# cipherflow-fhe/lattisense

Measured on AMD Instinct MI355X. Metric: ckks_hmult_relin_rescale_throughput, higher is better.
Workload: dtype u64

## Files before the change

### include/lattisense_amd.h

```cpp
#ifndef LATTISENSE_AMD_H
#define LATTISENSE_AMD_H
#include <stddef.h>
#include <stdint.h>

#ifdef __cplusplus
extern "C" {
#endif

typedef struct lsa_context_st* lsa_context;
typedef struct lsa_key_st* lsa_key;

enum { LSA_OK = 0, LSA_ERR_ARG = 1, LSA_ERR_NO_DEVICE = 2, LSA_ERR_HIP = 3, LSA_ERR_INTERNAL = 4 };
enum { LSA_ALGO_BFV = 0, LSA_ALGO_CKKS = 1 };

const char* lsa_last_error(void);
const char* lsa_version(void);
const char* lsa_build_flags(void);

int lsa_context_create(int algo, int n, const uint64_t* q, int nq, const uint64_t* p, int np, uint64_t t,
                       int device, lsa_context* out);
int lsa_context_destroy(lsa_context ctx);
int lsa_context_moduli(lsa_context ctx, uint64_t* out, int capacity, int* count);

int lsa_malloc(lsa_context ctx, void** dptr, size_t bytes);
// ... 79 lines not shown
                       void* stream);
int lsa_bfv_mult_sum(lsa_context ctx, int level, int n, const uint64_t* const* as, const long long* sas, const uint64_t* const* bs,
                     const long long* sbs, const uint64_t* addend, long long s_addend, uint64_t* d3, int batch, long long sd,
                     void* stream);
int lsa_bfv_dot(lsa_context ctx, int level, int n, const uint64_t* const* as, const long long* sas, const uint64_t* const* bs,
                const long long* sbs, const uint64_t* addend, long long s_addend, lsa_key rlk, uint64_t* out, int batch,
                long long sout, void* stream);
int lsa_bfv_dot_plan(int n_ring, const uint64_t* q, int nq, int level, int terms, int* max_terms, int* n_groups, int* aux_limbs);

int lsa_set_bfv_dot_chunk(lsa_context ctx, int pairs);
int lsa_set_tile_batch(lsa_context ctx, int tile_batch);
int lsa_set_fp64_ntt(lsa_context ctx, int enable);
int lsa_set_dual_stream(lsa_context ctx, int enable);
int lsa_set_fuse_tails(lsa_context ctx, int enable);
int lsa_set_modup_lift(lsa_context ctx, int enable);
int lsa_set_ks_tail_in_mac(lsa_context ctx, int mode);
int lsa_set_rescale_head_in_conv(lsa_context ctx, int mode);
int lsa_set_ntt_chunk_mib(lsa_context ctx, int mib);
int lsa_ckks_rotate_many(lsa_context ctx, int level, const uint64_t* in, int n_rot, const uint64_t* galois_elements,
                         const lsa_key* glk, uint64_t* const* outs, int batch, long long sin, long long sout, void* stream);
int lsa_bfv_rotate_many(lsa_context ctx, int level, const uint64_t* in, int n_rot, const uint64_t* galois_elements,
                        const lsa_key* glk, uint64_t* const* outs, int batch, long long sin, long long sout, void* stream);

typedef struct lsa_bootstrap_st* lsa_bootstrap;
int lsa_bootstrap_create(lsa_context ctx, int cts_depth, int stc_depth, int k, int double_angle, double message_ratio,
                         double in_scale, double out_scale, int log_slots, void* stream, lsa_bootstrap* out);
int lsa_bootstrap_create_ex(lsa_context ctx, int cts_depth, int stc_depth, int k, int double_angle, double message_ratio,
                            double in_scale, double out_scale, int log_slots, int sine_deg, int arcsine_deg, void* stream,
                            lsa_bootstrap* out);
int lsa_bootstrap_evalmod_constants(lsa_bootstrap b, int* n_cheb, double* cheb, int* n_asin, double* asin_coef);
// ... 115 lines not shown
```

### lattisense_amd/_native.py

```python
import ctypes
import importlib.util
import os

_HERE = os.path.dirname(os.path.abspath(__file__))
LIB_PATH = os.environ.get("LSA_NATIVE_LIB") or os.path.join(_HERE, "liblattisense_amd.so")

_lib = None

c_u64p = ctypes.POINTER(ctypes.c_uint64)
c_ll = ctypes.c_longlong
c_vp = ctypes.c_void_p
c_int = ctypes.c_int


class LsaError(RuntimeError):
    def __init__(self, code, msg):
        super().__init__("lattisense_amd error %d: %s" % (code, msg))
        self.code = code


def _preload_hip_runtime():
    spec = importlib.util.find_spec("torch")
    if spec is not None and spec.origin:
        p = os.path.join(os.path.dirname(spec.origin), "lib", "libamdhip64.so")
# ... 54 lines not shown
    "lsa_bfv_rotate": (c_int, [c_vp, c_int, c_vp, ctypes.c_uint64, c_vp, c_vp, c_int, c_ll, c_ll, c_vp]),
    "lsa_bfv_rescale": (c_int, [c_vp, c_int, c_int, c_vp, c_vp, c_int, c_ll, c_ll, c_vp]),
    "lsa_bfv_mult_relin": (c_int, [c_vp, c_int, c_vp, c_vp, c_vp, c_vp, c_int, c_ll, c_ll, c_ll, c_vp]),
    "lsa_bfv_mult_sum": (c_int, [c_vp, c_int, c_int, ctypes.POINTER(c_vp), ctypes.POINTER(c_ll), ctypes.POINTER(c_vp),
                                 ctypes.POINTER(c_ll), c_vp, c_ll, c_vp, c_int, c_ll, c_vp]),
    "lsa_bfv_dot": (c_int, [c_vp, c_int, c_int, ctypes.POINTER(c_vp), ctypes.POINTER(c_ll), ctypes.POINTER(c_vp), ctypes.POINTER(c_ll),
                            c_vp, c_ll, c_vp, c_vp, c_int, c_ll, c_vp]),
    "lsa_bfv_dot_plan": (c_int, [c_int, c_u64p, c_int, c_int, c_int, ctypes.POINTER(c_int), ctypes.POINTER(c_int),
                                 ctypes.POINTER(c_int)]),
    "lsa_set_bfv_dot_chunk": (c_int, [c_vp, c_int]),
    "lsa_set_tile_batch": (c_int, [c_vp, c_int]),
    "lsa_set_fp64_ntt": (c_int, [c_vp, c_int]),
    "lsa_set_dual_stream": (c_int, [c_vp, c_int]),
    "lsa_set_fuse_tails": (c_int, [c_vp, c_int]),
    "lsa_set_modup_lift": (c_int, [c_vp, c_int]),
    "lsa_set_ks_tail_in_mac": (c_int, [c_vp, c_int]),
    "lsa_set_rescale_head_in_conv": (c_int, [c_vp, c_int]),
    "lsa_set_ntt_chunk_mib": (c_int, [c_vp, c_int]),
    "lsa_debug_set_ntt_stamps": (c_int, [c_vp, c_vp]),
    "lsa_debug_baseconv_plans": (c_int, [c_vp, c_int, ctypes.POINTER(c_int), ctypes.POINTER(c_int), ctypes.POINTER(c_int),
                                         ctypes.POINTER(c_int)]),
    "lsa_debug_key_switch_fused": (c_int, [c_vp, c_int, c_vp, ctypes.POINTER(c_int)]),
    "lsa_ckks_rotate_many": (c_int, [c_vp, c_int, c_vp, c_int, c_u64p, ctypes.POINTER(c_vp), ctypes.POINTER(c_vp), c_int,
                                     ctypes.c_longlong, ctypes.c_longlong, c_vp]),
    "lsa_bfv_rotate_many": (c_int, [c_vp, c_int, c_vp, c_int, c_u64p, ctypes.POINTER(c_vp), ctypes.POINTER(c_vp), c_int,
                                    ctypes.c_longlong, ctypes.c_longlong, c_vp]),
    "lsa_bfv_mult_plain_mul": (c_int, [c_vp, c_int, c_vp, c_vp, c_vp, c_int, c_ll, c_ll, c_ll, c_vp]),
    "lsa_bfv_mac_plain_mul": (c_int, [c_vp, c_int, c_int, ctypes.POINTER(c_vp), ctypes.POINTER(c_ll), ctypes.POINTER(c_vp),
                                      ctypes.POINTER(c_ll), c_vp, c_ll, c_vp, c_int, c_ll, c_vp]),
    "lsa_bfv_rotate_mac_plain_mul": (c_int, [c_vp, c_int, c_vp, c_int, c_u64p, ctypes.POINTER(c_vp), ctypes.POINTER(c_vp),
# ... 112 lines not shown
```

### lattisense_amd/build.py

```python
import importlib.util
import os
import subprocess
import sys

HERE = os.path.dirname(os.path.abspath(__file__))
CSRC = os.path.join(HERE, "csrc")
LIB = os.path.join(HERE, "liblattisense_amd.so")
HIP_SOURCES = ["kernels.hip", "context.hip", "key_switch.hip", "ops.hip", "linear_transform.hip", "bfv_encode.hip", "bfv_plain.hip", "slot_sum.hip", "poly_eval.hip", "bfv_poly.hip", "bootstrap.hip", "c_api.hip", "task_runtime.hip", "task_transfer.hip",
               "task_dispatch.hip", "task_frontend.hip"]
CXX_SOURCES = ["tables.cpp", "task_graph.cpp"]
HEADERS = ["build_flags.h", "modarith.h", "ntt_core.h", "ntt_r16.h", "ntt_plan.h", "ntt_chunk.h", "tables.h", "lsa_internal.h", "linear_transform.h", "bfv_encode.h", "poly_eval.h", "bfv_poly.h", "poly_lincomb.h", "tensor_sum.h", "ks_mac_multi.h", "ks_mac_groups.h", "slot_sum.h", "galois_keys.h", "key_switch.h", "entry_check.h", "plain_ops.h", "bfv_plain.h", "layout_check.h", "task_graph.h", "mini_json.h", "buf_pool.h", "switches.h", "shard_plan.h", "task_pipeline.h", "task_internal.h",
           "../../include/lattisense_amd.h", "../../include/lattisense_task.h"]


def torch_lib_dir():
    spec = importlib.util.find_spec("torch")
    if spec is None or spec.origin is None:
        return None
    d = os.path.join(os.path.dirname(spec.origin), "lib")
    return d if os.path.exists(os.path.join(d, "libamdhip64.so")) else None


def _stale(target, deps):
    if not os.path.exists(target):
        return True
    t = os.path.getmtime(target)
# ... 25 lines not shown
        tl = torch_lib_dir()
        libdirs = ([tl] if tl else []) + ["/opt/rocm/lib"]
        cmd = ["g++", "-shared", "-Wl,-soname,liblattisense_amd.so", "-o", LIB] + objs
        for d in libdirs:
            cmd += ["-L" + d, "-Wl,-rpath," + d]
        cmd += ["-lamdhip64", "-lpthread"]
        if verbose:
            print(" ".join(cmd), file=sys.stderr)
        subprocess.check_call(cmd)
    return LIB


def build_variant(name, flags, verbose=False):
    hipcc = os.environ.get("HIPCC", "/opt/rocm/bin/hipcc")
    build_native()
    diag = any(t in flags for t in ("_DIAG_NO_", "_DIAG_COPY_ONLY", "_DIAG_COMPUTE_ONLY", "_DIAG_TW8"))
    if diag and "-DLSA_DIAG_BUILD" not in flags:
        flags = flags + " -DLSA_DIAG_BUILD"
    flags = flags + " -DLSA_VARIANT_NAME=" + name
    vdir = os.path.join(HERE, "variants")
    objdir = os.path.join(CSRC, "build", "variant_" + name)
    os.makedirs(vdir, exist_ok=True)
    os.makedirs(objdir, exist_ok=True)
    hdrs = [os.path.join(CSRC, h) for h in HEADERS]
    hdr_text = "".join(open(h).read() for h in hdrs if os.path.exists(h))
    macros = [f[2:].split("=")[0] for f in flags.split() if f.startswith("-D")]
    objs = []
    for src in [s for s in HIP_SOURCES + CXX_SOURCES if os.path.exists(os.path.join(CSRC, s))]:
        sp = os.path.join(CSRC, src)
        base_obj = os.path.join(CSRC, "build", src.replace(".", "_") + ".o")
        text = open(sp).read()
# ... 32 lines not shown
```

### lattisense_amd/csrc/build_flags.h

```cpp
#pragma once

#if (defined(LSA_NTT_DIAG_NO_TWIDDLE_LOADS) || defined(LSA_NTT_DIAG_COPY_ONLY) || defined(LSA_NTT_DIAG_COMPUTE_ONLY) || defined(LSA_NTT_DIAG_TW8) || \
     defined(LSA_KS_DIAG_NO_MATH) || defined(LSA_KS_DIAG_NO_STORE) || defined(LSA_BC_DIAG_NO_MATH) || defined(LSA_BC_DIAG_NO_STORE)) && \
    !defined(LSA_DIAG_BUILD)
#error "wrong-result diagnostic switches need -DLSA_DIAG_BUILD (use lattisense_amd.build --variant: it adds the flag and renames the library)"
#endif

#define LSA_BF_STR2(x) #x
#define LSA_BF_STR(x) LSA_BF_STR2(x)

#define LSA_BUILD_FLAGS_TEXT_1 ""
#ifdef LSA_DIAG_BUILD
#define LSA_BF_DIAG " LSA_DIAG_BUILD"
#else
#define LSA_BF_DIAG ""
#endif
#ifdef LSA_NTT_DIAG_NO_TWIDDLE_LOADS
#define LSA_BF_A " LSA_NTT_DIAG_NO_TWIDDLE_LOADS"
#else
#define LSA_BF_A ""
#endif
#ifdef LSA_NTT_DIAG_COPY_ONLY
#define LSA_BF_B " LSA_NTT_DIAG_COPY_ONLY"
#else
// ... 137 lines not shown
#if defined(LSA_KSMAC_TWCACHE) && LSA_KSMAC_TWCACHE != 1
#define LSA_BF_AH " LSA_KSMAC_TWCACHE=" LSA_BF_STR(LSA_KSMAC_TWCACHE)
#else
#define LSA_BF_AH ""
#endif
#ifdef LSA_NTT_DIAG_TW8
#define LSA_BF_AD " LSA_NTT_DIAG_TW8"
#else
#define LSA_BF_AD ""
#endif
#ifdef LSA_LIFT_ROW_OUTER
#define LSA_BF_AG " LSA_LIFT_ROW_OUTER"
#else
#define LSA_BF_AG ""
#endif
#ifdef LSA_VARIANT_NAME
#define LSA_BF_V " variant=" LSA_BF_STR(LSA_VARIANT_NAME)
#else
#define LSA_BF_V ""
#endif
#ifdef LSA_AB_SWITCH
#define LSA_BF_W " LSA_AB_SWITCH=" LSA_BF_STR(LSA_AB_SWITCH)
#else
#define LSA_BF_W ""
#endif

#define LSA_BUILD_FLAGS_TEXT                                                                                              \
    LSA_BF_DIAG LSA_BF_A LSA_BF_B LSA_BF_C LSA_BF_D LSA_BF_E LSA_BF_F LSA_BF_G LSA_BF_H LSA_BF_I LSA_BF_J LSA_BF_K LSA_BF_L \
        LSA_BF_M LSA_BF_N LSA_BF_O LSA_BF_P LSA_BF_Q LSA_BF_R LSA_BF_S LSA_BF_T LSA_BF_U LSA_BF_V LSA_BF_W LSA_BF_X LSA_BF_Y LSA_BF_Z LSA_BF_AA LSA_BF_AB LSA_BF_AC LSA_BF_AD LSA_BF_AE LSA_BF_AF LSA_BF_AG LSA_BF_AH
```

### lattisense_amd/csrc/c_api.hip

```cpp
#include "bfv_encode.h"
#include "bfv_poly.h"
#include "build_flags.h"
#include "linear_transform.h"
#include "poly_eval.h"
#include "lsa_internal.h"

namespace lsa {
const char* kernels_build_flags();
const char* context_build_flags();
}

using namespace lsa;

struct lsa_context_st {
    Context ctx;
    lsa_context_st(int algo, int n, const u64* q, int nq, const u64* p, int np, u64 t, int dev)
        : ctx(algo, n, q, nq, p, np, t, dev) {}
};
struct lsa_key_st {
    Key key;
    double* fp_owned = nullptr;
};

template <typename F>
// ... 423 lines not shown
        Context& c = C(ctx);
        LSA_REQUIRE(kind >= 0 && kind < LSA_PROF_KINDS && total_bytes_primary, "bad argument");
        double by = 0;
        for (auto& sm : c.prof_samples)
            if (sm.kid == kind) by += sm.bytes_primary;
        *total_bytes_primary = by;
    });
}

int lsa_set_fuse_tails(lsa_context ctx, int enable) {
    return guard([&] { C(ctx).fuse_tails = enable ? 1 : 0; });
}
int lsa_set_modup_lift(lsa_context ctx, int enable) {
    return guard([&] { C(ctx).modup_lift = enable ? 1 : 0; });
}
int lsa_set_ks_tail_in_mac(lsa_context ctx, int mode) {
    return guard([&] {
        LSA_REQUIRE(mode >= 0 && mode <= 2, "lsa_set_ks_tail_in_mac: mode is 0, 1 or 2");
        C(ctx).ks_tail_in_mac = mode;
    });
}
int lsa_set_rescale_head_in_conv(lsa_context ctx, int mode) {
    return guard([&] {
        LSA_REQUIRE(mode >= 0 && mode <= 2, "lsa_set_rescale_head_in_conv: mode is 0, 1 or 2");
        C(ctx).rescale_head_in_conv = mode;
    });
}
int lsa_set_dual_stream(lsa_context ctx, int enable) {
    return guard([&] { C(ctx).dual_stream = enable ? 1 : 0; });
}
// ... 595 lines not shown
```

### lattisense_amd/csrc/emu_ntt.cpp

```cpp
#define LSA_EMULATE 1
#include <cstddef>
#include <vector>
#include "ntt_plan.h"
#include "ntt_chunk.h"
#include "ntt_r16.h"
#include <array>
#include "tables.h"

template <int NT>
static void emu_block(const NttPassArgs& a, const NttBlockCtx& bc, u64* lds) {
    for (int t = 0; t < NT; t++) ntt_phase_load<true, NT, true>(a, bc, t, lds);
    int rho[4];
    const int np = ntt_split(a.mu, rho);
    if (!a.inverse) {
        int sig = 0;
        for (int i = 0; i < np; i++) {
            for (int t = 0; t < NT; t++) ntt_phase_sub_dyn<NT>(a, bc, t, lds, sig, rho[i]);
            sig += rho[i];
        }
    } else {
        int sig = a.mu;
        for (int i = np - 1; i >= 0; i--) {
            sig -= rho[i];
            for (int t = 0; t < NT; t++) ntt_phase_sub_dyn<NT>(a, bc, t, lds, sig, rho[i]);
        }
    }
    for (int t = 0; t < NT; t++) ntt_phase_store<true, NT>(a, bc, t, lds);
}

template <int PASS, int MU, int FZ = 3 | 16>
static void emu_block_r16(const NttPassArgs& a, const NttBlockCtx& bc, u64* lds) {
    std::vector<std::array<u64, 16>> regs(LSA_R16_THREADS);
    for (int phase = 0; phase < 3; phase++)
        for (int t = 0; t < LSA_R16_THREADS; t++) {
            u64(&v)[16] = *reinterpret_cast<u64(*)[16]>(regs[t].data());
            r16_phase<PASS, FZ, MU>(a, bc, t, lds, phase, v);
        }
}

static void emu_block_r8x3(const NttPassArgs& a, const NttBlockCtx& bc, u64* lds) {
    std::vector<std::array<u64, 16>> regs(LSA_R16_THREADS);
    for (int phase = 0; phase < 4; phase++)
        for (int t = 0; t < LSA_R16_THREADS; t++) {
            u64(&v)[16] = *reinterpret_cast<u64(*)[16]>(regs[t].data());
            r8x3_phase<3 | 16>(a, bc, t, lds, phase, v);
        }
}

static int emu_ntt(int n, const u64* moduli, int nmod, u64* data, int batch, long long batch_stride, int rows,
                   const unsigned char* mod_of, int period, int inverse, int tau_max, int allow_fp64, const u64* pa, const u64* pb,
                   const u64* lift = nullptr, int lift_mod = 0, int lift_limbs = 1, int chunk = 0, long long sa = -1,
                   long long sb = -1, long long slift = -1) {
    const int row_inner = (allow_fp64 >> 1) & 1;
    const bool r16 = (allow_fp64 >> 2) & 1;
    allow_fp64 &= 1;
    lsa::HostTables T;
    T.build(n, std::vector<u64>(moduli, moduli + nmod));
    NttPlan plan = make_ntt_plan(T.logn, tau_max);
    std::vector<u64> tw_i(T.psi.size());
    std::vector<double> tw_d(T.psi_d.size());
    for (int m = 0; m < nmod; m++) {
        const size_t o = (size_t)m * n;
        ntt_permute_twiddles(plan, T.logn, (inverse ? T.psiinv : T.psi).data() + 2 * o, tw_i.data() + 2 * o, 2, false);
        ntt_permute_twiddles(plan, T.logn, (inverse ? T.psiinv_d : T.psi_d).data() + o, tw_d.data() + o, 1, true);
    }
    NttPassArgs a{};
    a.src = data;
// ... 38 lines not shown
    const NttPassArgs whole = a;
    const int items = chunk > 0 && chunk < batch ? chunk : batch;
    for (int b0 = 0; b0 < batch; b0 += items) {
        const int nb = batch - b0 < items ? batch - b0 : items;
        a = ntt_chunk_rebase(whole, b0);
        a.batch = nb;
        a.src = a.dst = data + (long long)b0 * batch_stride;
        for (int step = 0; step < plan.npass; step++) {
            int k = inverse ? plan.npass - 1 - step : step;
            ntt_fill_pass(a, plan, T.logn, k, inverse);
            a.fz_first = step == 0;
            a.fp_raw_out = plan.npass == 2 && step == 0;
            a.fp_raw_in = plan.npass == 2 && step == 1;
            std::vector<u64> lds(lds_words(a.tau));
            long long nblocks = (long long)nb * launch_rows * (1 << (a.logn - a.tau));
            for (long long bid = 0; bid < nblocks; bid++) {
                NttBlockCtx bc = ntt_decode_block(a, bid);
                if (bc.mod == LSA_ROW_SKIP) continue;
                if (r16 && ntt_r16_shape_ok(a, plan.npass)) {
                    if (a.mu == 9) emu_block_r8x3(a, bc, lds.data());
                    else if (a.lambda && lift) (a.mu == 8 ? emu_block_r16<0, 8, 32> : emu_block_r16<0, 7, 32>)(a, bc, lds.data());
                    else if (a.lambda && a.mu == 8) emu_block_r16<0, 8>(a, bc, lds.data());
                    else if (a.lambda) emu_block_r16<0, 7>(a, bc, lds.data());
                    else if (a.mu == 8) emu_block_r16<1, 8>(a, bc, lds.data());
                    else emu_block_r16<1, 7>(a, bc, lds.data());
                } else if (a.tau <= 12) emu_block<LSA_NTT_THREADS>(a, bc, lds.data());
                else if (a.tau == 13) emu_block<512>(a, bc, lds.data());
                else emu_block<1024>(a, bc, lds.data());
            }
        }
// ... 24 lines not shown
extern "C" int lsa_emu_intt_prod_chunked(int n, const u64* moduli, int nmod, const u64* pa, long long sa, const u64* pb, long long sb,
                                         u64* out, int batch, long long batch_stride, int rows, const unsigned char* mod_of,
                                         int period, int tau_max, int allow_fp64, int chunk) {
    if (!pa || !pb || sa < 0 || sb < 0 || chunk < 0) return -1;
    return emu_ntt(n, moduli, nmod, out, batch, batch_stride, rows, mod_of, period, 1, tau_max, allow_fp64, pa, pb, nullptr, 0, 1,
                   chunk, sa, sb);
}

extern "C" int lsa_emu_ntt_lift_chunked(int n, const u64* moduli, int nmod, const u64* src, long long src_stride, int src_mod,
                                        int limbs, u64* out, int batch, long long batch_stride, int rows,
                                        const unsigned char* mod_of, int period, int tau_max, int allow_fp64, int chunk) {
    if (!src || src_stride < 0 || limbs < 1 || rows % limbs || src_mod < 0 || src_mod + rows / limbs > nmod || chunk < 0) return -1;
    return emu_ntt(n, moduli, nmod, out, batch, batch_stride, rows, mod_of, period, 0, tau_max, allow_fp64, nullptr, nullptr, src,
                   src_mod, limbs, chunk, -1, -1, src_stride);
}
```

### lattisense_amd/csrc/kernels.hip

```cpp
#include <atomic>
#include <cstdlib>

#include "build_flags.h"
#include "ks_mac_groups.h"
#include "lsa_internal.h"
#include "ntt_r16.h"
#include "plain_ops.h"
#include "poly_lincomb.h"
#include "tensor_sum.h"

namespace lsa {

const char* kernels_build_flags() { return LSA_BUILD_FLAGS_TEXT; }

static constexpr int TPB = 256;

#ifndef LSA_NTT_WAVES
#define LSA_NTT_WAVES 4
#endif

#if defined(LSA_NTT_DIAG_STAMPS)
#define LSA_STAMP(k)                                                                               \
    do {                                                                                           \
        if (a.diag && threadIdx.x == 0 && blockIdx.x < 8192) a.diag[blockIdx.x * 8 + (k)] = __builtin_amdgcn_s_memtime(); \
// ... 97 lines not shown
#endif
template <int PASS, int FZ, int MU>
__global__ __launch_bounds__(LSA_R16_THREADS, (FZ & 1) ? LSA_NTT_WAVES_FUSED : LSA_R16_WAVES) void k_ntt_r16(NttPassArgs a) {
    extern __shared__ __attribute__((aligned(16))) u64 lds[];
    const int tid = threadIdx.x;
    const NttBlockCtx bc = ntt_decode_block(a, (long long)blockIdx.x);
    if (bc.mod == LSA_ROW_SKIP) return;
    u64 v[16];
    r16_phase<PASS, FZ, MU>(a, bc, tid, lds, 0, v);
    if (!(PASS == 0 && a.inverse)) r16_sync<PASS>();
    r16_phase<PASS, FZ, MU>(a, bc, tid, lds, 1, v);
    if (PASS == 0 && !a.inverse) return;
    r16_sync<PASS>();
    r16_phase<PASS, FZ, MU>(a, bc, tid, lds, 2, v);
}
template <int FZ>
__global__ __launch_bounds__(LSA_R16_THREADS, LSA_R16_WAVES) void k_ntt_r8x3(NttPassArgs a) {
    extern __shared__ __attribute__((aligned(16))) u64 lds[];
    const int tid = threadIdx.x;
    const NttBlockCtx bc = ntt_decode_block(a, (long long)blockIdx.x);
    if (bc.mod == LSA_ROW_SKIP) return;
    u64 v[16];
    r8x3_phase<FZ>(a, bc, tid, lds, 0, v);
    r16_sync<1>();
    r8x3_phase<FZ>(a, bc, tid, lds, 1, v);
    r16_sync<1>();
    r8x3_phase<FZ>(a, bc, tid, lds, 2, v);
    r16_sync<1>();
    r8x3_phase<FZ>(a, bc, tid, lds, 3, v);
}
static int ntt_pass_fz(const NttPassArgs& a, bool fused) {
    const bool pro = fused && a.fz_pro && a.fz_first, epi = fused && a.fz_epi && a.final_reduce;
    if (pro && a.fz_pro == 3) return 16;
    if (epi && a.fz_epi == 3) return 4;
    if (epi && a.fz_epi == 4) return 8;
    return (pro ? 1 : 0) | (epi ? 2 : 0);
}
template <int FZ>
static auto ntt_r16_second_pass(int mu) {
    return mu == 9 ? &k_ntt_r8x3<FZ> : mu == 8 ? &k_ntt_r16<1, FZ, 8> : &k_ntt_r16<1, FZ, 7>;
}
static bool ntt_launch_r16(const NttPassArgs& a, int npass, bool fused, long long nblocks, hipStream_t s) {
    if (!sw::ntt_r16() || !ntt_r16_shape_ok(a, npass)) return false;
    const int fz = ntt_pass_fz(a, fused);
    void (*k)(NttPassArgs) = nullptr;
    if (a.lambda) {
        if (fz == 1 && a.fz_pro == 4 && sw::r16_pro()) k = a.mu == 8 ? &k_ntt_r16<0, 32, 8> : &k_ntt_r16<0, 32, 7>;
        else if (fz == 1 && a.fz_pro != 4 && a.mu == 8 && sw::r16_pro()) k = &k_ntt_r16<0, 1, 8>;
        else if (fz == 0) k = a.mu == 8 ? &k_ntt_r16<0, 0, 8> : &k_ntt_r16<0, 0, 7>;
    } else if (a.mu != 9 || sw::ntt_r8x3()) {
        switch (fz) {
            case 0: k = ntt_r16_second_pass<0>(a.mu); break;
            case 2: k = ntt_r16_second_pass<2>(a.mu); break;
            case 4: k = ntt_r16_second_pass<4>(a.mu); break;
            case 8: k = ntt_r16_second_pass<8>(a.mu); break;
            case 16: k = a.inverse ? ntt_r16_second_pass<16>(a.mu) : nullptr; break;
        }
    }
    if (!k) return false;
// ... 351 lines not shown
        a.fz_b_stride = fz->b_stride;
        a.fz_b_rpp = fz->b_rpp;
    }
    a.period = rm.period;
    a.row0 = rm.row0;
    a.row_step = rm.row_step;
    for (int i = 0; i < rm.period; i++) {
        LSA_REQUIRE(rm.mod_of[i] == LSA_ROW_SKIP || rm.mod_of[i] < c.nmod, "ntt: modulus index out of range");
        a.mod_of[i] = rm.mod_of[i];
    }
    int active_rows = 0;
    for (int r = 0; r < rows; r++) active_rows += rm.mod_of[(rm.row0 + r * rm.row_step) % rm.period] != LSA_ROW_SKIP;
    if (active_rows == 0) return;
    int launch_rows = rows;
    a.compact = 0;
    if (active_rows <= LSA_MAX_PERIOD && rm.row0 + (rows - 1) * rm.row_step < 65536) {
        a.compact = 1;
        int k = 0;
        for (int r = 0; r < rows; r++) {
            const int row = rm.row0 + r * rm.row_step;
            if (rm.mod_of[row % rm.period] != LSA_ROW_SKIP) a.row_tbl[k++] = (unsigned short)row;
        }
        launch_rows = active_rows;
    }
    a.rows = launch_rows;
    bool wide = c.plan_wide.npass < c.plan.npass && c.wide_mode != 0;
    if (wide && c.wide_mode == 2) {
        bool all_fp = c.fp64_ntt != 0;
        for (int r = 0; r < rows && all_fp; r++) {
            const unsigned char m = rm.mod_of[(rm.row0 + r * rm.row_step) % rm.period];
            if (m != LSA_ROW_SKIP && (c.T.mods[m].q >> LSA_FP64_MAX_BITS) != 0) all_fp = false;
        }
        const long long limbs = (long long)active_rows * batch;
        wide = !fz && (c.logn == 13 ? limbs >= 1024 : (all_fp && limbs >= 512));
    }
    if (passes != 3) wide = false;
// ... 31 lines not shown
            const int k = inverse ? plan.npass - 1 - step : step;
            ntt_fill_pass(a, plan, c.logn, k, inverse ? 1 : 0);
            a.fp_raw_out = plan.npass == 2 && step == 0 && c.fp_raw;
            a.fp_raw_in = plan.npass == 2 && step == 1 && c.fp_raw;
            LSA_REQUIRE(!(a.fz_first && a.fz_pro && a.fp_raw_in), "ntt: a fused prologue reads canonical inputs, never a raw hand-off");
            a.src = (step == 0 ? src + (long long)b0 * src_stride : dst + (long long)b0 * dst_stride);
            a.src_stride = step == 0 ? src_stride : dst_stride;
            a.dst = dst + (long long)b0 * dst_stride;
            a.dst_stride = dst_stride;
            a.total_tiles = (long long)nb * launch_rows * (1 << (a.logn - a.tau));
            const long long nblocks = a.total_tiles;
            LSA_REQUIRE(nblocks < (1LL << 31), "ntt: grid too large");
            const size_t lds_bytes = (size_t)lds_words(a.tau) * sizeof(u64);
            const double pro_bytes = fz && fz->pro == 3 && a.fz_first ? 8.0 * c.n * active_rows * nb : 0.0;
            ProfScope ps(c, PROF_NTT, 16.0 * c.n * active_rows * nb / plan.npass + pro_bytes, s);
            if (ntt_launch_r16(a, plan.npass, fz != nullptr, nblocks, s)) continue;
            if (a.tau <= 12) ntt_launch_pass<LSA_NTT_THREADS>(a, fz != nullptr, nblocks, lds_bytes, s);
            else if (a.tau == 13) ntt_launch_pass<512>(a, fz != nullptr, nblocks, lds_bytes, s);
            else ntt_launch_pass<1024>(a, fz != nullptr, nblocks, lds_bytes, s);
        }
    }
}

struct EwArgs {
    const u64* a;
    const u64* b;
    const u64* acc;
    u64* out;
    long long sa, sb, so, sacc;
    const ModDev* mods;
    int rows, logn, op, period;
// ... 1984 lines not shown
```

### lattisense_amd/csrc/lsa_internal.h

```cpp
#pragma once
#include <hip/hip_runtime.h>
#include <cstdint>
#include <map>
#include <memory>
#include <mutex>
#include <stdexcept>
#include <string>
#include <vector>

#include "../../include/lattisense_amd.h"
#include "galois_keys.h"
#include "ntt_plan.h"
#include "ntt_chunk.h"
#include "plain_ops.h"
#include "slot_sum.h"
#include "switches.h"
#include "tables.h"

namespace lsa {

void set_last_error(const std::string& m);

#define LSA_HIP(expr)                                                                                     \
    do {                                                                                                  \
// ... 57 lines not shown
    int wide_mode = 2;
    ModDev* d_mods = nullptr;
    u64* d_psi = nullptr;
    u64* d_psiinv = nullptr;
    u64* d_scale = nullptr;
    double* d_psi_d = nullptr;
    double* d_psiinv_d = nullptr;
    u64* d_psi_w = nullptr;
    u64* d_psiinv_w = nullptr;
    double* d_psi_d_w = nullptr;
    double* d_psiinv_d_w = nullptr;
    double* d_scale_d = nullptr;
    int fp64_ntt = 1;
    int tile_batch = 0;
    int fp_raw = 1;
    int modup_lift = 1;
    int fuse_tails = 1;
    int ks_tail_in_mac = 1;
    int rescale_head_in_conv = 1;
    int dual_stream = 0;
    hipStream_t aux_stream = nullptr;
    hipEvent_t ev_fork = nullptr, ev_join = nullptr;
    void fork_aux(hipStream_t s);
    void join_aux(hipStream_t s);
    unsigned long long* ntt_diag = nullptr;
    int ntt_chunk_mib = 0;
    int bfv_dot_chunk = 0;

    struct ProfSample {
        hipEvent_t e0, e1;
// ... 396 lines not shown
```

### lattisense_amd/csrc/ntt_r16.h

```cpp
#pragma once
#include "ntt_core.h"

#define LSA_R16_THREADS 256
#define LSA_R16_LDS_WORDS (272 * 16)

LSA_HD bool ntt_r16_shape_ok(const NttPassArgs& a, int npass) {
    if (npass != 2 || a.tau != 12) return false;
    if (a.mu == 9) return a.s_lo == a.logn - 9 && a.lambda == 0;
    if (a.mu != 8 && a.mu != 7) return false;
    return (a.s_lo == 0 && a.lambda == 12 - a.mu) || (a.s_lo == a.logn - a.mu && a.lambda == 0);
}

template <int PASS, int MU>
LSA_HD int r16_lds(int k, int i) {
    const int p = i + (i >> 4);
    return PASS == 0 ? (p << (12 - MU)) + k : k * ((1 << MU) + (1 << (MU - 4))) + p;
}
template <int PASS, int MU>
LSA_HD long long r16_x(const NttPassArgs& a, int tile, int k, int i) {
    return PASS == 0 ? ((long long)tile << (12 - MU)) + ((long long)i << (a.logn - MU)) + k : ((long long)tile << 12) + (k << MU) + i;
}
template <int MU, int IMAGE>
LSA_HD int r16_pt(int i, int e) {
    return IMAGE == 0 ? i + (e << (MU - 4)) : 16 * i + e;
// ... 98 lines not shown
            }
            if (f.fp_lift) {
#pragma unroll
                for (int e = 8 * h; e < 8 * h + 8; e++) {
                    const double td = u52_to_double(t[e]);
                    const double r = td > f.hd ? td - f.qld : td;
                    v[e] = d_to_bits(u52_to_double(v[e]) + r);
                }
            } else {
#pragma unroll
                for (int e = 8 * h; e < 8 * h + 8; e++) v[e] = ntt_load_fix(f, v[e], t[e]);
            }
        }
        return;
    }
#pragma unroll
    for (int e = 0; e < 16; e++) v[e] = r16_load1(g + r16_x<PASS, MU>(a, bc.tile, k, r16_pt<MU, IMAGE>(i, e)));
    if (FZ && LIFT != 0 && f.lift) {
        ntt_lift_block<16>(f, v);
        return;
    }
    if (!(FZ && LIFT != 2 && f.head)) {
        if (f.fp && !f.raw) {
#pragma unroll
            for (int e = 0; e < 16; e++) v[e] = d_to_bits(u52_to_double(v[e]));
        }
        return;
    }
    NttLoadFix f1 = f;
    f1.add = false;
#pragma unroll
    for (int e = 0; e < 16; e++) v[e] = ntt_load_fix(f1, v[e], v[e]);
// ... 300 lines not shown
            r16_store_coalesced<(FZ & 2) != 0, MU, (FZ & 4) != 0, (FZ & 8) != 0>(a, bc, tid, lds);
        }
    } else {
        if (phase == 0) {
            if (PASS == 0) r16_load_direct<PASS, false, 1, MU>(a, bc, tid, v);
            else r16_load_coalesced<false, MU, (FZ & 16) != 0>(a, bc, tid, lds);
        } else if (phase == 1) {
            if (PASS == 1) r16_lds_get<PASS, 1, MU>(tid, lds, v);
            r16_group<PASS, 1, MU>(v, a, bc, L, G2);
            r16_lds_put<PASS, 1, MU>(tid, lds, v);
        } else {
            r16_lds_get<PASS, 0, MU>(tid, lds, v);
            r16_group<PASS, 0, MU>(v, a, bc, L, G1);
            r16_store_direct<PASS, false, 0, MU>(a, bc, tid, v);
        }
    }
}

template <int IMAGE>
LSA_HD int r8x3_pt(int i, int E) {
    if (IMAGE == 0) return i + (E << 5);
    if (IMAGE == 2) return 16 * i + E;
    return ((2 * (i >> 3) + (E >> 3)) << 6) | ((E & 7) << 3) | (i & 7);
}
template <int IMAGE>
LSA_HD constexpr int r8x3_slot(int g, int e) {
    return IMAGE == 0 ? g + 2 * e : 8 * g + e;
}
template <int IMAGE>
LSA_HD void r8x3_group(u64 (&v)[16], const NttPassArgs& a, const NttBlockCtx& bc, const R16Limb& L, unsigned G1, int i) {
// ... 346 lines not shown
```

### lattisense_amd/device.py

```python
import ctypes

import numpy as np

from . import _native
from ._native import check, lib

ALGO_BFV, ALGO_CKKS = 0, 1


class DeviceBuffer:
    def __init__(self, ctx, nwords):
        self.ctx = ctx
        self.nwords = int(nwords)
        p = ctypes.c_void_p()
        check(lib().lsa_malloc(ctx.h, ctypes.byref(p), self.nwords * 8))
        self.ptr = p.value

    def free(self):
        if self.ptr:
            check(lib().lsa_free(self.ctx.h, self.ptr))
            self.ptr = None

    def __del__(self):
        try:
# ... 56 lines not shown
    def baseconv_plans(self):
        cnt = ctypes.c_int()
        check(lib().lsa_debug_baseconv_plans(self.h, 0, ctypes.byref(cnt), None, None, None))
        n = cnt.value
        ns, nd, sp = (ctypes.c_int * max(n, 1))(), (ctypes.c_int * max(n, 1))(), (ctypes.c_int * max(n, 1))()
        check(lib().lsa_debug_baseconv_plans(self.h, n, ctypes.byref(cnt), ns, nd, sp))
        return [(ns[i], nd[i], bool(sp[i])) for i in range(min(n, cnt.value))]

    def key_switch_fused(self, level, key):
        out = ctypes.c_int()
        check(lib().lsa_debug_key_switch_fused(self.h, level, key, ctypes.byref(out)))
        return bool(out.value)

    def set_modup_lift(self, enable):
        check(lib().lsa_set_modup_lift(self.h, int(enable)))

    def set_ks_tail_in_mac(self, mode):
        check(lib().lsa_set_ks_tail_in_mac(self.h, int(mode)))

    def set_rescale_head_in_conv(self, mode):
        check(lib().lsa_set_rescale_head_in_conv(self.h, int(mode)))

    def set_bfv_dot_chunk(self, pairs):
        check(lib().lsa_set_bfv_dot_chunk(self.h, int(pairs)))

    def set_fp64_ntt(self, enable):
        check(lib().lsa_set_fp64_ntt(self.h, int(enable)))

    def upload_key(self, compact, key_level):
        compact = np.ascontiguousarray(compact, dtype=np.uint64)
# ... 718 lines not shown
```

Baseline: 16250.

## Add walk NTT kernel that reuses one loaded source tile across lifted rows

Adds a fused NTT first-pass kernel for the modup-lift case. Each block loads the source limb tile into registers once, then walks several target rows of the same polynomial, lifting and transforming each one. Rows are grouped by fp64/integer engine class into units. Before this, every output row was its own block that reloaded the same source data. The kernel is on by default (lift_walk=-1 means all rows of a polynomial in one unit), so there are fewer blocks and fewer redundant global loads, at the cost of serial work per block, lower parallelism and more register pressure from holding the kept source.

```diff
diff --git a/include/lattisense_amd.h b/include/lattisense_amd.h
--- a/include/lattisense_amd.h
+++ b/include/lattisense_amd.h
@@ -117,6 +117,8 @@
 int lsa_set_dual_stream(lsa_context ctx, int enable);
 int lsa_set_fuse_tails(lsa_context ctx, int enable);
 int lsa_set_modup_lift(lsa_context ctx, int enable);
+int lsa_set_lift_walk(lsa_context ctx, int rows_per_unit);
+int lsa_debug_lift_walk(lsa_context ctx, int* rows_per_unit, long long* launches);
 int lsa_set_ks_tail_in_mac(lsa_context ctx, int mode);
 int lsa_set_rescale_head_in_conv(lsa_context ctx, int mode);
 int lsa_set_ntt_chunk_mib(lsa_context ctx, int mib);
diff --git a/lattisense_amd/_native.py b/lattisense_amd/_native.py
--- a/lattisense_amd/_native.py
+++ b/lattisense_amd/_native.py
@@ -92,6 +92,8 @@
     "lsa_set_dual_stream": (c_int, [c_vp, c_int]),
     "lsa_set_fuse_tails": (c_int, [c_vp, c_int]),
     "lsa_set_modup_lift": (c_int, [c_vp, c_int]),
+    "lsa_set_lift_walk": (c_int, [c_vp, c_int]),
+    "lsa_debug_lift_walk": (c_int, [c_vp, ctypes.POINTER(c_int), ctypes.POINTER(c_ll)]),
     "lsa_set_ks_tail_in_mac": (c_int, [c_vp, c_int]),
     "lsa_set_rescale_head_in_conv": (c_int, [c_vp, c_int]),
     "lsa_set_ntt_chunk_mib": (c_int, [c_vp, c_int]),
diff --git a/lattisense_amd/build.py b/lattisense_amd/build.py
--- a/lattisense_amd/build.py
+++ b/lattisense_amd/build.py
@@ -9,7 +9,7 @@
 HIP_SOURCES = ["kernels.hip", "context.hip", "key_switch.hip", "ops.hip", "linear_transform.hip", "bfv_encode.hip", "bfv_plain.hip", "slot_sum.hip", "poly_eval.hip", "bfv_poly.hip", "bootstrap.hip", "c_api.hip", "task_runtime.hip", "task_transfer.hip",
                "task_dispatch.hip", "task_frontend.hip"]
 CXX_SOURCES = ["tables.cpp", "task_graph.cpp"]
-HEADERS = ["build_flags.h", "modarith.h", "ntt_core.h", "ntt_r16.h", "ntt_plan.h", "ntt_chunk.h", "tables.h", "lsa_internal.h", "linear_transform.h", "bfv_encode.h", "poly_eval.h", "bfv_poly.h", "poly_lincomb.h", "tensor_sum.h", "ks_mac_multi.h", "ks_mac_groups.h", "slot_sum.h", "galois_keys.h", "key_switch.h", "entry_check.h", "plain_ops.h", "bfv_plain.h", "layout_check.h", "task_graph.h", "mini_json.h", "buf_pool.h", "switches.h", "shard_plan.h", "task_pipeline.h", "task_internal.h",
+HEADERS = ["build_flags.h", "modarith.h", "ntt_core.h", "ntt_r16.h", "ntt_plan.h", "ntt_chunk.h", "ntt_walk.h", "tables.h", "lsa_internal.h", "linear_transform.h", "bfv_encode.h", "poly_eval.h", "bfv_poly.h", "poly_lincomb.h", "tensor_sum.h", "ks_mac_multi.h", "ks_mac_groups.h", "slot_sum.h", "galois_keys.h", "key_switch.h", "entry_check.h", "plain_ops.h", "bfv_plain.h", "layout_check.h", "task_graph.h", "mini_json.h", "buf_pool.h", "switches.h", "shard_plan.h", "task_pipeline.h", "task_internal.h",
            "../../include/lattisense_amd.h", "../../include/lattisense_task.h"]
 
 
@@ -65,7 +65,7 @@
 def build_variant(name, flags, verbose=False):
     hipcc = os.environ.get("HIPCC", "/opt/rocm/bin/hipcc")
     build_native()
-    diag = any(t in flags for t in ("_DIAG_NO_", "_DIAG_COPY_ONLY", "_DIAG_COMPUTE_ONLY", "_DIAG_TW8"))
+    diag = any(t in flags for t in ("_DIAG_NO_", "_DIAG_COPY_ONLY", "_DIAG_COMPUTE_ONLY", "_DIAG_TW8", "_DIAG_LIFT_NO_"))
     if diag and "-DLSA_DIAG_BUILD" not in flags:
         flags = flags + " -DLSA_DIAG_BUILD"
     flags = flags + " -DLSA_VARIANT_NAME=" + name
diff --git a/lattisense_amd/csrc/build_flags.h b/lattisense_amd/csrc/build_flags.h
--- a/lattisense_amd/csrc/build_flags.h
+++ b/lattisense_amd/csrc/build_flags.h
@@ -1,7 +1,8 @@
 #pragma once
 
 #if (defined(LSA_NTT_DIAG_NO_TWIDDLE_LOADS) || defined(LSA_NTT_DIAG_COPY_ONLY) || defined(LSA_NTT_DIAG_COMPUTE_ONLY) || defined(LSA_NTT_DIAG_TW8) || \
-     defined(LSA_KS_DIAG_NO_MATH) || defined(LSA_KS_DIAG_NO_STORE) || defined(LSA_BC_DIAG_NO_MATH) || defined(LSA_BC_DIAG_NO_STORE)) && \
+     defined(LSA_KS_DIAG_NO_MATH) || defined(LSA_KS_DIAG_NO_STORE) || defined(LSA_BC_DIAG_NO_MATH) || defined(LSA_BC_DIAG_NO_STORE) || \
+     defined(LSA_NTT_DIAG_LIFT_NO_LOAD)) && \
     !defined(LSA_DIAG_BUILD)
 #error "wrong-result diagnostic switches need -DLSA_DIAG_BUILD (use lattisense_amd.build --variant: it adds the flag and renames the library)"
 #endif
@@ -175,6 +176,21 @@
 #else
 #define LSA_BF_AG ""
 #endif
+#ifdef LSA_NTT_DIAG_LIFT_NO_LOAD
+#define LSA_BF_AI " LSA_NTT_DIAG_LIFT_NO_LOAD"
+#else
+#define LSA_BF_AI ""
+#endif
+#if defined(LSA_WALK_SRC) && LSA_WALK_SRC != 0
+#define LSA_BF_AJ " LSA_WALK_SRC=" LSA_BF_STR(LSA_WALK_SRC)
+#else
+#define LSA_BF_AJ ""
+#endif
+#ifdef LSA_WALK_WAVES
+#define LSA_BF_AK " LSA_WALK_WAVES=" LSA_BF_STR(LSA_WALK_WAVES)
+#else
+#define LSA_BF_AK ""
+#endif
 #ifdef LSA_VARIANT_NAME
 #define LSA_BF_V " variant=" LSA_BF_STR(LSA_VARIANT_NAME)
 #else
@@ -188,4 +204,4 @@
 
 #define LSA_BUILD_FLAGS_TEXT                                                                                              \
     LSA_BF_DIAG LSA_BF_A LSA_BF_B LSA_BF_C LSA_BF_D LSA_BF_E LSA_BF_F LSA_BF_G LSA_BF_H LSA_BF_I LSA_BF_J LSA_BF_K LSA_BF_L \
-        LSA_BF_M LSA_BF_N LSA_BF_O LSA_BF_P LSA_BF_Q LSA_BF_R LSA_BF_S LSA_BF_T LSA_BF_U LSA_BF_V LSA_BF_W LSA_BF_X LSA_BF_Y LSA_BF_Z LSA_BF_AA LSA_BF_AB LSA_BF_AC LSA_BF_AD LSA_BF_AE LSA_BF_AF LSA_BF_AG LSA_BF_AH
+        LSA_BF_M LSA_BF_N LSA_BF_O LSA_BF_P LSA_BF_Q LSA_BF_R LSA_BF_S LSA_BF_T LSA_BF_U LSA_BF_V LSA_BF_W LSA_BF_X LSA_BF_Y LSA_BF_Z LSA_BF_AA LSA_BF_AB LSA_BF_AC LSA_BF_AD LSA_BF_AE LSA_BF_AF LSA_BF_AG LSA_BF_AH LSA_BF_AI LSA_BF_AJ LSA_BF_AK
diff --git a/lattisense_amd/csrc/c_api.hip b/lattisense_amd/csrc/c_api.hip
--- a/lattisense_amd/csrc/c_api.hip
+++ b/lattisense_amd/csrc/c_api.hip
@@ -461,6 +461,19 @@
 int lsa_set_modup_lift(lsa_context ctx, int enable) {
     return guard([&] { C(ctx).modup_lift = enable ? 1 : 0; });
 }
+int lsa_set_lift_walk(lsa_context ctx, int rows_per_unit) {
+    return guard([&] {
+        LSA_REQUIRE(rows_per_unit >= -1, "lsa_set_lift_walk: -1 (the launcher's rule), 0 (per-row launch) or rows per unit");
+        C(ctx).lift_walk = rows_per_unit;
+    });
+}
+int lsa_debug_lift_walk(lsa_context ctx, int* rows_per_unit, long long* launches) {
+    return guard([&] {
+        Context& c = C(ctx);
+        if (rows_per_unit) *rows_per_unit = c.lift_walk;
+        if (launches) *launches = c.lift_walk_launches.load(std::memory_order_relaxed);
+    });
+}
 int lsa_set_ks_tail_in_mac(lsa_context ctx, int mode) {
     return guard([&] {
         LSA_REQUIRE(mode >= 0 && mode <= 2, "lsa_set_ks_tail_in_mac: mode is 0, 1 or 2");
diff --git a/lattisense_amd/csrc/emu_ntt.cpp b/lattisense_amd/csrc/emu_ntt.cpp
--- a/lattisense_amd/csrc/emu_ntt.cpp
+++ b/lattisense_amd/csrc/emu_ntt.cpp
@@ -4,6 +4,7 @@
 #include "ntt_plan.h"
 #include "ntt_chunk.h"
 #include "ntt_r16.h"
+#include "ntt_walk.h"
 #include <array>
 #include "tables.h"
 
@@ -38,6 +39,24 @@
         }
 }
 
+template <int MU, bool KEEP>
+static void emu_walk_block(const NttPassArgs& a, const NttWalkUnits& u, long long bid, u64* lds) {
+    const NttWalkBlock blk = ntt_walk_decode(bid, u.n_units, a.batch);
+    const int first = u.first[blk.unit], count = u.count[blk.unit];
+    std::vector<std::array<u64, 16>> src(LSA_R16_THREADS), regs(LSA_R16_THREADS);
+    if (KEEP)
+        for (int t = 0; t < LSA_R16_THREADS; t++)
+            r16_walk_load<MU>(a, ntt_walk_block_ctx(a, blk.b, u.row[first], blk.tile), t, *reinterpret_cast<u64(*)[16]>(src[t].data()));
+    for (int r = 0; r < count; r++) {
+        const NttBlockCtx bc = ntt_walk_block_ctx(a, blk.b, u.row[first + r], blk.tile);
+        LSA_EMU_CHECK((bc.fp != 0) == (u.cls[blk.unit] != 0));
+        for (int phase = 0; phase < 2; phase++)
+            for (int t = 0; t < LSA_R16_THREADS; t++)
+                r16_walk_phase<MU, KEEP>(a, bc, t, lds, phase, *reinterpret_cast<const u64(*)[16]>(src[t].data()),
+                                         *reinterpret_cast<u64(*)[16]>(regs[t].data()));
+    }
+}
+
 static void emu_block_r8x3(const NttPassArgs& a, const NttBlockCtx& bc, u64* lds) {
     std::vector<std::array<u64, 16>> regs(LSA_R16_THREADS);
     for (int phase = 0; phase < 4; phase++)
@@ -50,7 +69,7 @@
 static int emu_ntt(int n, const u64* moduli, int nmod, u64* data, int batch, long long batch_stride, int rows,
                    const unsigned char* mod_of, int period, int inverse, int tau_max, int allow_fp64, const u64* pa, const u64* pb,
                    const u64* lift = nullptr, int lift_mod = 0, int lift_limbs = 1, int chunk = 0, long long sa = -1,
-                   long long sb = -1, long long slift = -1) {
+                   long long sb = -1, long long slift = -1, int walk = -1, bool walk_keep = true) {
     const int row_inner = (allow_fp64 >> 1) & 1;
     const bool r16 = (allow_fp64 >> 2) & 1;
     allow_fp64 &= 1;
@@ -119,6 +138,19 @@
             a.fp_raw_in = plan.npass == 2 && step == 1;
             std::vector<u64> lds(lds_words(a.tau));
             long long nblocks = (long long)nb * launch_rows * (1 << (a.logn - a.tau));
+            NttWalkUnits wu;
+            if (lift && walk >= 0 && a.fz_first && a.lambda && r16 && ntt_r16_shape_ok(a, plan.npass)) {
+                unsigned char row_fp[LSA_MAX_PERIOD];
+                for (int i = 0; i < a.rows; i++)
+                    row_fp[i] = allow_fp64 && (T.mods[mod_of[a.row_tbl[i] % period]].q >> LSA_FP64_MAX_BITS) == 0;
+                if (!ntt_walk_units(a.row_tbl, a.rows, a.fz_limbs, walk, row_fp, wu)) return -2;
+                const long long wblocks = ntt_walk_blocks(wu.n_units, a.batch, 1 << (a.logn - a.tau));
+                for (long long bid = 0; bid < wblocks; bid++) {
+                    if (a.mu == 8) (walk_keep ? emu_walk_block<8, true> : emu_walk_block<8, false>)(a, wu, bid, lds.data());
+                    else (walk_keep ? emu_walk_block<7, true> : emu_walk_block<7, false>)(a, wu, bid, lds.data());
+                }
+                continue;
+            }
             for (long long bid = 0; bid < nblocks; bid++) {
                 NttBlockCtx bc = ntt_decode_block(a, bid);
                 if (bc.mod == LSA_ROW_SKIP) continue;
@@ -173,3 +205,12 @@
     return emu_ntt(n, moduli, nmod, out, batch, batch_stride, rows, mod_of, period, 0, tau_max, allow_fp64, nullptr, nullptr, src,
                    src_mod, limbs, chunk, -1, -1, src_stride);
 }
+
+extern "C" int lsa_emu_ntt_lift_walk(int n, const u64* moduli, int nmod, const u64* src, long long src_stride, int src_mod, int limbs,
+                                     u64* out, int batch, long long batch_stride, int rows, const unsigned char* mod_of, int period,
+                                     int tau_max, int allow_fp64, int chunk, int walk, int keep) {
+    if (!src || src_stride < 0 || limbs < 1 || rows % limbs || src_mod < 0 || src_mod + rows / limbs > nmod || chunk < 0 || walk < 0) return -1;
+    if (!((allow_fp64 >> 2) & 1)) return -2;
+    return emu_ntt(n, moduli, nmod, out, batch, batch_stride, rows, mod_of, period, 0, tau_max, allow_fp64, nullptr, nullptr, src,
+                   src_mod, limbs, chunk, -1, -1, src_stride, walk, keep != 0);
+}
diff --git a/lattisense_amd/csrc/kernels.hip b/lattisense_amd/csrc/kernels.hip
--- a/lattisense_amd/csrc/kernels.hip
+++ b/lattisense_amd/csrc/kernels.hip
@@ -5,6 +5,7 @@
 #include "ks_mac_groups.h"
 #include "lsa_internal.h"
 #include "ntt_r16.h"
+#include "ntt_walk.h"
 #include "plain_ops.h"
 #include "poly_lincomb.h"
 #include "tensor_sum.h"
@@ -135,6 +136,50 @@
     r16_sync<PASS>();
     r16_phase<PASS, FZ, MU>(a, bc, tid, lds, 2, v);
 }
+#ifndef LSA_WALK_SRC
+#define LSA_WALK_SRC 0
+#endif
+#ifndef LSA_WALK_WAVES
+#define LSA_WALK_WAVES (LSA_WALK_SRC == 0 ? LSA_NTT_WAVES_FUSED : LSA_R16_WAVES)
+#endif
+static_assert(LSA_WALK_MAX_UNITS == LSA_MAX_PERIOD, "a walk launch has at most one unit per active row");
+struct NttWalkArgs {
+    NttPassArgs a;
+    NttWalkUnits u;
+};
+template <int MU, bool KEEP, bool FP>
+__device__ __forceinline__ void r16_walk_rows(const NttWalkArgs& w, const NttWalkBlock& blk, int first, int count, int tid, u64* lds, u64 (&src)[16]) {
+    const NttPassArgs& a = w.a;
+    for (int r = 0; r < count; r++) {
+        NttBlockCtx bc = ntt_walk_block_ctx(a, blk.b, w.u.row[first + r], blk.tile);
+        bc.fp = FP ? 1 : 0;
+        u64 v[16];
+        int t0 = tid, t1 = tid;
+        asm volatile("" : "+v"(t0));
+        if (KEEP) {
+#pragma unroll
+            for (int e = 0; e < 16; e++) asm volatile("" : "+v"(src[e]));
+        }
+        r16_walk_phase<MU, KEEP>(a, bc, t0, lds, 0, src, v);
+        __syncthreads();
+        asm volatile("" : "+v"(t1));
+        r16_walk_phase<MU, KEEP>(a, bc, t1, lds, 1, src, v);
+        if (r + 1 < count) __syncthreads();
+    }
+}
+template <int MU>
+__global__ __launch_bounds__(LSA_R16_THREADS, LSA_WALK_WAVES) void k_ntt_r16_walk(NttWalkArgs w) {
+    extern __shared__ __attribute__((aligned(16))) u64 lds[];
+    constexpr bool KEEP = LSA_WALK_SRC == 0;
+    const int tid = threadIdx.x;
+    const NttPassArgs& a = w.a;
+    const NttWalkBlock blk = ntt_walk_decode((long long)blockIdx.x, w.u.n_units, a.batch);
+    const int first = w.u.first[blk.unit], count = w.u.count[blk.unit];
+    u64 src[16];
+    if (KEEP) r16_walk_load<MU>(a, ntt_walk_block_ctx(a, blk.b, w.u.row[first], blk.tile), tid, src);
+    if (w.u.cls[blk.unit]) r16_walk_rows<MU, KEEP, true>(w, blk, first, count, tid, lds, src);
+    else r16_walk_rows<MU, KEEP, false>(w, blk, first, count, tid, lds, src);
+}
 template <int FZ>
 __global__ __launch_bounds__(LSA_R16_THREADS, LSA_R16_WAVES) void k_ntt_r8x3(NttPassArgs a) {
     extern __shared__ __attribute__((aligned(16))) u64 lds[];
@@ -161,9 +206,23 @@
 static auto ntt_r16_second_pass(int mu) {
     return mu == 9 ? &k_ntt_r8x3<FZ> : mu == 8 ? &k_ntt_r16<1, FZ, 8> : &k_ntt_r16<1, FZ, 7>;
 }
-static bool ntt_launch_r16(const NttPassArgs& a, int npass, bool fused, long long nblocks, hipStream_t s) {
+static constexpr int LIFT_WALK_RULE = 0;
+static bool ntt_launch_r16(const NttPassArgs& a, int npass, bool fused, long long nblocks, hipStream_t s, int lift_walk = 0,
+                           const unsigned char* row_fp = nullptr, bool* walked = nullptr) {
     if (!sw::ntt_r16() || !ntt_r16_shape_ok(a, npass)) return false;
     const int fz = ntt_pass_fz(a, fused);
+    if (a.lambda && fz == 1 && a.fz_pro == 4 && sw::r16_pro() && lift_walk != 0 && a.compact && row_fp) {
+        NttWalkArgs w;
+        if (ntt_walk_units(a.row_tbl, a.rows, a.fz_limbs, lift_walk > 0 ? lift_walk : LIFT_WALK_RULE, row_fp, w.u)) {
+            w.a = a;
+            const long long nb = ntt_walk_blocks(w.u.n_units, a.batch, 1 << (a.logn - a.tau));
+            void (*kw)(NttWalkArgs) = a.mu == 8 ? &k_ntt_r16_walk<8> : &k_ntt_r16_walk<7>;
+            hipLaunchKernelGGL(kw, dim3((unsigned)nb), dim3(LSA_R16_THREADS), (size_t)LSA_R16_LDS_WORDS * sizeof(u64), s, w);
+            LSA_HIP(hipGetLastError());
+            if (walked) *walked = true;
+            return true;
+        }
+    }
     void (*k)(NttPassArgs) = nullptr;
     if (a.lambda) {
         if (fz == 1 && a.fz_pro == 4 && sw::r16_pro()) k = a.mu == 8 ? &k_ntt_r16<0, 32, 8> : &k_ntt_r16<0, 32, 7>;
@@ -545,12 +604,16 @@
     if (active_rows == 0) return;
     int launch_rows = rows;
     a.compact = 0;
+    unsigned char row_fp[LSA_MAX_PERIOD];
     if (active_rows <= LSA_MAX_PERIOD && rm.row0 + (rows - 1) * rm.row_step < 65536) {
         a.compact = 1;
         int k = 0;
         for (int r = 0; r < rows; r++) {
             const int row = rm.row0 + r * rm.row_step;
-            if (rm.mod_of[row % rm.period] != LSA_ROW_SKIP) a.row_tbl[k++] = (unsigned short)row;
+            const unsigned char m = rm.mod_of[row % rm.period];
+            if (m == LSA_ROW_SKIP) continue;
+            row_fp[k] = c.fp_engine(m) ? 1 : 0;
+            a.row_tbl[k++] = (unsigned short)row;
         }
         launch_rows = active_rows;
     }
@@ -612,7 +675,10 @@
             const size_t lds_bytes = (size_t)lds_words(a.tau) * sizeof(u64);
             const double pro_bytes = fz && fz->pro == 3 && a.fz_first ? 8.0 * c.n * active_rows * nb : 0.0;
             ProfScope ps(c, PROF_NTT, 16.0 * c.n * active_rows * nb / plan.npass + pro_bytes, s);
-            if (ntt_launch_r16(a, plan.npass, fz != nullptr, nblocks, s)) continue;
+            bool walked = false;
+            const bool r16 = ntt_launch_r16(a, plan.npass, fz != nullptr, nblocks, s, c.lift_walk, a.compact ? row_fp : nullptr, &walked);
+            if (walked) c.lift_walk_launches.fetch_add(1, std::memory_order_relaxed);
+            if (r16) continue;
             if (a.tau <= 12) ntt_launch_pass<LSA_NTT_THREADS>(a, fz != nullptr, nblocks, lds_bytes, s);
             else if (a.tau == 13) ntt_launch_pass<512>(a, fz != nullptr, nblocks, lds_bytes, s);
             else ntt_launch_pass<1024>(a, fz != nullptr, nblocks, lds_bytes, s);
diff --git a/lattisense_amd/csrc/lsa_internal.h b/lattisense_amd/csrc/lsa_internal.h
--- a/lattisense_amd/csrc/lsa_internal.h
+++ b/lattisense_amd/csrc/lsa_internal.h
@@ -1,5 +1,6 @@
 #pragma once
 #include <hip/hip_runtime.h>
+#include <atomic>
 #include <cstdint>
 #include <map>
 #include <memory>
@@ -95,6 +96,8 @@
     int fp64_ntt = 1;
     int tile_batch = 0;
     int fp_raw = 1;
+    int lift_walk = -1;
+    std::atomic<long long> lift_walk_launches{0};
     int modup_lift = 1;
     int fuse_tails = 1;
     int ks_tail_in_mac = 1;
diff --git a/lattisense_amd/csrc/ntt_r16.h b/lattisense_amd/csrc/ntt_r16.h
--- a/lattisense_amd/csrc/ntt_r16.h
+++ b/lattisense_amd/csrc/ntt_r16.h
@@ -136,8 +136,13 @@
         }
         return;
     }
-#pragma unroll
-    for (int e = 0; e < 16; e++) v[e] = r16_load1(g + r16_x<PASS, MU>(a, bc.tile, k, r16_pt<MU, IMAGE>(i, e)));
+#if defined(LSA_NTT_DIAG_LIFT_NO_LOAD)
+    constexpr bool no_load = FZ && LIFT == 2;
+#else
+    constexpr bool no_load = false;
+#endif
+#pragma unroll
+    for (int e = 0; e < 16; e++) v[e] = no_load ? (u64)(k + 16 * e + 1) : r16_load1(g + r16_x<PASS, MU>(a, bc.tile, k, r16_pt<MU, IMAGE>(i, e)));
     if (FZ && LIFT != 0 && f.lift) {
         ntt_lift_block<16>(f, v);
         return;
@@ -468,6 +473,55 @@
             r16_group<PASS, 0, MU>(v, a, bc, L, G1);
             r16_store_direct<PASS, false, 0, MU>(a, bc, tid, v);
         }
+    }
+}
+
+LSA_HD NttBlockCtx ntt_walk_block_ctx(const NttPassArgs& a, int b, int row, int tile) {
+    NttBlockCtx c;
+    c.tile = tile;
+    c.base_src = (long long)b * a.src_stride + ((long long)row << a.logn);
+    c.base_dst = (long long)b * a.dst_stride + ((long long)row << a.logn);
+    c.mod = a.mod_of[row % a.period];
+    c.b = b;
+    c.row = row;
+    c.tw_l = nullptr;
+    c.fp = a.allow_fp64 && (a.mods[c.mod].q >> LSA_FP64_MAX_BITS) == 0;
+    return c;
+}
+template <int MU>
+LSA_HD void r16_walk_load(const NttPassArgs& a, const NttBlockCtx& bc, int tid, u64 (&src)[16]) {
+    const u64* g;
+    const u64* gl;
+    ntt_make_load_fix<true, 2>(a, bc, g, gl);
+    int k, i;
+    r16_lane<0, MU>(tid, k, i);
+#pragma unroll
+    for (int e = 0; e < 16; e++) src[e] = r16_load1(g + r16_x<0, MU>(a, bc.tile, k, r16_pt<MU, 0>(i, e)));
+}
+template <int MU, bool KEEP>
+LSA_HD void r16_walk_phase(const NttPassArgs& a, const NttBlockCtx& bc, int tid, u64* lds, int phase, const u64 (&src)[16], u64 (&v)[16]) {
+    const R16Limb L = r16_limb(a, bc);
+    int k, i;
+    r16_lane<0, MU>(tid, k, i);
+    const unsigned G1 = r16_G1<0, MU>(bc, k), G2 = (G1 << 4) + ((unsigned)i << (8 - MU));
+    if (phase == 0) {
+        if (KEEP) {
+            const u64* g;
+            const u64* gl;
+            const NttLoadFix f = ntt_make_load_fix<true, 2>(a, bc, g, gl);
+            LSA_EMU_CHECK(f.lift);
+#pragma unroll
+            for (int e = 0; e < 16; e++) v[e] = src[e];
+            ntt_lift_block<16>(f, v);
+        } else {
+            r16_load_direct<0, true, 0, MU, 2>(a, bc, tid, v);
+        }
+        r16_group<0, 0, MU>(v, a, bc, L, G1);
+        r16_lds_put<0, 0, MU>(tid, lds, v);
+    } else {
+        r16_lds_get<0, 1, MU>(tid, lds, v);
+        r16_group<0, 1, MU>(v, a, bc, L, G2);
+        r16_store_direct<0, false, 1, MU>(a, bc, tid, v);
     }
 }
 
diff --git a/lattisense_amd/csrc/ntt_walk.h b/lattisense_amd/csrc/ntt_walk.h
--- /dev/null
+++ b/lattisense_amd/csrc/ntt_walk.h
@@ -0,0 +1,62 @@
+#pragma once
+
+#if defined(__HIPCC__)
+#define LSA_WALK_HD __host__ __device__ inline
+#else
+#define LSA_WALK_HD inline
+#endif
+
+#define LSA_WALK_MAX_UNITS 192
+#define LSA_WALK_MAX_ROWS 255
+
+struct NttWalkUnits {
+    int n_units;
+    unsigned short row[LSA_WALK_MAX_UNITS];
+    unsigned short first[LSA_WALK_MAX_UNITS];
+    unsigned char count[LSA_WALK_MAX_UNITS];
+    unsigned char cls[LSA_WALK_MAX_UNITS];
+};
+
+inline bool ntt_walk_units(const unsigned short* row_tbl, int n_rows, int fz_limbs, int walk, const unsigned char* cls, NttWalkUnits& u) {
+    u.n_units = 0;
+    if (n_rows < 1 || n_rows > LSA_WALK_MAX_UNITS || fz_limbs < 1) return false;
+    if (walk <= 0 || walk > LSA_WALK_MAX_ROWS) walk = LSA_WALK_MAX_ROWS;
+    for (int r = 1; r < n_rows; r++)
+        if (row_tbl[r] <= row_tbl[r - 1]) return false;
+    int i = 0, out = 0;
+    while (i < n_rows) {
+        const int poly = row_tbl[i] / fz_limbs;
+        int j = i + 1;
+        while (j < n_rows && row_tbl[j] / fz_limbs == poly) j++;
+        for (int c = 1; c >= 0; c--) {
+            const int begin = out;
+            for (int r = i; r < j; r++)
+                if ((cls && cls[r] ? 1 : 0) == c) u.row[out++] = row_tbl[r];
+            const int n = out - begin, parts = (n + walk - 1) / walk;
+            int at = begin;
+            for (int p = 0; p < parts; p++) {
+                const int len = n / parts + (p < n % parts ? 1 : 0);
+                u.first[u.n_units] = (unsigned short)at;
+                u.count[u.n_units] = (unsigned char)len;
+                u.cls[u.n_units] = (unsigned char)c;
+                u.n_units++;
+                at += len;
+            }
+        }
+        i = j;
+    }
+    return true;
+}
+
+struct NttWalkBlock {
+    int tile, unit, b;
+};
+LSA_WALK_HD NttWalkBlock ntt_walk_decode(long long bid, int n_units, int batch) {
+    NttWalkBlock w;
+    w.b = (int)(bid % batch);
+    const long long ut = bid / batch;
+    w.unit = (int)(ut % n_units);
+    w.tile = (int)(ut / n_units);
+    return w;
+}
+inline long long ntt_walk_blocks(int n_units, int batch, int tiles) { return (long long)tiles * n_units * batch; }
diff --git a/lattisense_amd/device.py b/lattisense_amd/device.py
--- a/lattisense_amd/device.py
+++ b/lattisense_amd/device.py
@@ -94,6 +94,14 @@
 
     def set_modup_lift(self, enable):
         check(lib().lsa_set_modup_lift(self.h, int(enable)))
+
+    def set_lift_walk(self, rows_per_unit):
+        check(lib().lsa_set_lift_walk(self.h, int(rows_per_unit)))
+
+    def lift_walk_launches(self):
+        n = ctypes.c_longlong()
+        check(lib().lsa_debug_lift_walk(self.h, None, ctypes.byref(n)))
+        return n.value
 
     def set_ks_tail_in_mac(self, mode):
         check(lib().lsa_set_ks_tail_in_mac(self.h, int(mode)))
```

Result: no change. 16460 (median of 6 runs) (+1.3%).
